# NikolayKrivosheev/Distributed-deep-learning-on-personal-computers

Hardware: AMD Instinct MI355X
Metric: images/sec (whole node), U-Net 256x256 6-class tiles (higher is better)
Workload: dtype bf16

## Files before the change

### csrc/bindings.cpp

```cpp
#include <ATen/ATen.h>
#include <c10/core/DeviceGuard.h>
#include <c10/hip/HIPStream.h>
#include <torch/library.h>

#include <cstdlib>
#include <mutex>
#include <string>
#include <unordered_map>
#include <vector>

#include "ops.h"

namespace ddlpc {

namespace {

hipStream_t cur_stream() { return c10::hip::getCurrentHIPStream().stream(); }

#define CHECK_DEV(t) TORCH_CHECK((t).is_cuda(), #t " must be a GPU tensor")
#define CHECK_CONTIG(t) TORCH_CHECK((t).is_contiguous(), #t " must be contiguous")
#define CHECK_BF16(t) TORCH_CHECK((t).scalar_type() == at::kBFloat16, #t " must be bf16")
#define CHECK_F32(t) TORCH_CHECK((t).scalar_type() == at::kFloat, #t " must be fp32")

const bf16_t* bptr(const at::Tensor& t) { return reinterpret_cast<const bf16_t*>(t.data_ptr()); }
bf16_t* bptr_mut(at::Tensor& t) { return reinterpret_cast<bf16_t*>(t.data_ptr()); }
const float* fptr_opt(const c10::optional<at::Tensor>& t) {
  return (t.has_value() && t->defined()) ? t->data_ptr<float>() : nullptr;
}

struct Geo {
  int dims, N, D, H, W, C;
};
Geo geo_of(const at::Tensor& x) {
  TORCH_CHECK(x.dim() == 4 || x.dim() == 5, "expected [N,(D,)H,W,C] channel-last tensor");
  Geo g;
  g.dims = (int)x.dim() - 2;
  g.N = (int)x.size(0);
  g.D = g.dims == 3 ? (int)x.size(1) : 1;
  g.H = (int)x.size(g.dims == 3 ? 2 : 1);
  g.W = (int)x.size(g.dims == 3 ? 3 : 2);
  g.C = (int)x.size(-1);
  return g;
}
std::vector<int64_t> shape_with_c(const Geo& g, int C, int scale = 1) {
  if (g.dims == 2) return {g.N, (int64_t)g.H * scale, (int64_t)g.W * scale, C};
  return {g.N, (int64_t)g.D * scale, (int64_t)g.H * scale, (int64_t)g.W * scale, C};
}

int pow2ceil(int v) { int p = 1; while (p < v) p <<= 1; return p; }

void conv_tile(int dims, int BM, int W, int& TD, int& TH, int& TW) {
  if (dims == 2) {
    TD = 1;
    TW = W >= 16 ? 16 : 8;
    TH = BM / TW;
  } else {
    TW = W >= 16 ? 16 : 8;
    TH = 4;
    TD = BM / (TW * TH);
  }
}

int pick_bn(int Cout) {
  if (Cout <= 32) return 32;
  if (Cout <= 64) return 64;
  return 128;
}

}

namespace {
thread_local std::string g_last_path;
}
void set_last_path(const std::string& path) { g_last_path = path; }
std::string last_path() { return g_last_path; }

namespace {
const char* const kKnobs[] = {"CROP_LDS_T", "WINDOW_LDS_T"};
bool knob_registered(const std::string& name) {
  for (const char* k : kKnobs)
    if (k[0] != 0 && name == k) return true;
  return false;
}
std::mutex g_knob_mu;
std::unordered_map<std::string, int>& knob_map() {
  static std::unordered_map<std::string, int> m;
  return m;
}
}

int knob(const char* name, int def) {
  TORCH_CHECK(knob_registered(name), "knob '", name, "' read but not listed in kKnobs");
  std::lock_guard<std::mutex> lk(g_knob_mu);
  auto& m = knob_map();
  auto it = m.find(name);
  if (it != m.end()) return it->second;
  const std::string env = std::string("DDLPC_") + name;
  const char* e = getenv(env.c_str());
  const int v = e ? atoi(e) : def;
  m.emplace(name, v);
  return v;
}

namespace {

int64_t set_knob(const std::string& name, int64_t value) {
  TORCH_CHECK(knob_registered(name), "set_knob: no kernel reads a knob named '", name,
              "' (registered knobs are listed in kKnobs, csrc/bindings.cpp)");
  std::lock_guard<std::mutex> lk(g_knob_mu);
  auto& m = knob_map();
  auto it = m.find(name);
  const int64_t prev = it != m.end() ? it->second : INT64_MIN;
  if (value == INT64_MIN) {
    if (it != m.end()) m.erase(it);
  } else {
    m[name] = (int)value;
  }
  return prev;
}

int phys_cus() {
  static int n = -1;
  if (n < 0) {
    hipDeviceProp_t prop;
    int dev = 0;
    hipGetDevice(&dev);
    n = (hipGetDeviceProperties(&prop, dev) == hipSuccess) ? prop.multiProcessorCount : 256;
  }
  return n;
}

int g_cu_reserve = 0;

int num_cus() { return std::max(8, phys_cus() - g_cu_reserve); }

at::Tensor reduce_rows(const at::Tensor& partial, int64_t R, int64_t N) {
  auto dopts = partial.options().dtype(at::kDouble);
  at::Tensor sums = at::empty({N}, dopts);
  const int RC = reduce_rows_chunks((int)R);
  at::Tensor tmp = RC > 1 ? at::empty({2 * RC * N}, dopts) : sums;
  reduce_rows_launch(partial.data_ptr<float>(), (int)R, N, tmp.data_ptr<double>(),
                     sums.data_ptr<double>(), cur_stream());
  return sums;
}

std::vector<at::Tensor> conv3_fwd(const at::Tensor& x1, const c10::optional<at::Tensor>& x2,
                                  const at::Tensor& w, const c10::optional<at::Tensor>& bias,
                                  const c10::optional<at::Tensor>& pscale,
                                  const c10::optional<at::Tensor>& pshift, int64_t cout,
                                  int64_t co1, bool want_stats_in,
                                  const c10::optional<at::Tensor>& pscale2,
                                  const c10::optional<at::Tensor>& pshift2,
                                  const c10::optional<at::Tensor>& bnb_y,
                                  const c10::optional<at::Tensor>& bnb_s4, int64_t groups) {
  CHECK_DEV(x1); CHECK_CONTIG(x1); CHECK_BF16(x1); CHECK_BF16(w); CHECK_CONTIG(w);
  c10::DeviceGuard guard(x1.device());
  const Geo g = geo_of(x1);
  bool want_stats = want_stats_in;
  ConvFwdArgs a{};
  a.dims = g.dims; a.N = g.N; a.D = g.D; a.H = g.H; a.W = g.W;
  a.C1 = g.C;
// ... 702 lines not shown
  at::Tensor out = at::empty(shape_with_c(g, (int)cout, 2), x.options());
  a.C = out.data_ptr();
  const bool res = convt_res_launch(a, num_cus(), cur_stream());
  if (!res) gemm_launch(a, cur_stream());
  set_last_path(res ? "convt_fwd:res" : "convt_fwd:gemm");
  return out;
}

std::vector<at::Tensor> convt_dgrad(const at::Tensor& dout, const at::Tensor& wd, int64_t cin,
                                    const c10::optional<at::Tensor>& bny,
                                    const c10::optional<at::Tensor>& bn4) {
  CHECK_DEV(dout); CHECK_CONTIG(dout); CHECK_BF16(dout); CHECK_BF16(wd);
  c10::DeviceGuard guard(dout.device());
  const Geo go = geo_of(dout);
  Geo g = go;
  g.H /= 2; g.W /= 2; if (g.dims == 3) g.D /= 2;
  const int S = g.dims == 2 ? 4 : 8;
  GemmArgs a{};
  a.mode = GEMM_CONVT_DGRAD;
  a.M = g.N * g.D * g.H * g.W;
  a.N = (int)cin;
  a.K = S * go.C;
  a.A = bptr(dout);
  a.B = bptr(wd);
  a.dims = g.dims; a.Nimg = g.N; a.D = g.D; a.H = g.H; a.W = g.W;
  a.Cin = (int)cin; a.Cout = go.C;
  TORCH_CHECK(go.C % 32 == 0, "convT dgrad needs Cout % 32 == 0");
  TORCH_CHECK((int64_t)a.M * (g.dims == 2 ? 4 : 8) < (int64_t)INT32_MAX, "convT: too many pixels for 32-bit pixel indices");
  at::Tensor dx = at::empty(shape_with_c(g, (int)cin), dout.options());
  a.C = dx.data_ptr();
  at::Tensor bnpart = at::empty({0}, dout.options().dtype(at::kFloat));
  a.bn4 = bn4_ptr(bn4, (int)cin);
  if (a.bn4 != nullptr) {
    TORCH_CHECK(bny.has_value() && bny->defined() && bny->is_contiguous() &&
                bny->numel() == dx.numel() && bny->scalar_type() == at::kBFloat16,
                "convt_dgrad: bny must be the deferred pre-BN input (shape of dx, bf16)");
    a.bny = bptr(*bny);
  }
  const int res_rows = convt_res_rows(a, num_cus());
  if (a.bn4 != nullptr) {
    const long long grid = res_rows > 0 ? res_rows : gemm_nt_grid(a);
    bnpart = at::empty({(int64_t)grid, 2, (int64_t)cin}, dout.options().dtype(at::kFloat));
    a.bnpart = bnpart.data_ptr<float>();
  }
  const bool res = res_rows != 0 && convt_res_launch(a, num_cus(), cur_stream());
  if (!res) gemm_launch(a, cur_stream());
  set_last_path(res ? "convt_dgrad:res" : "convt_dgrad:gemm");
  return {dx, bnpart};
}

static at::Tensor convt_bias_grad(const at::Tensor& x, const at::Tensor& dout, const Geo& go,
                                  const c10::optional<at::Tensor>& colsum_rows,
                                  const c10::optional<at::Tensor>& db_out, bool into) {
  auto fopts = x.options().dtype(at::kFloat);
  at::Tensor db = into ? *db_out : at::empty({go.C}, fopts);
  if (colsum_rows.has_value() && colsum_rows->defined() && colsum_rows->numel() > 0) {
    const at::Tensor& cr = *colsum_rows;
    TORCH_CHECK(cr.dim() == 3 && cr.size(1) == 2 && cr.size(2) >= go.C, "colsum rows [R][2][C]");
    const int R = (int)cr.size(0);
    at::Tensor ctmp = R > 64 ? at::empty({(int64_t)((R + 63) / 64) * go.C}, x.options().dtype(at::kDouble))
                             : at::empty({0}, x.options().dtype(at::kDouble));
    reduce_rows_scatter_launch(cr.data_ptr<float>(), R, go.C, ctmp.data_ptr<double>(),
                               db.data_ptr<float>(), 2, 0, 0, 0, into, cur_stream(), 2 * cr.size(2));
  } else {
    const long long P = (long long)go.N * go.D * go.H * go.W;
    const int nb = (int)std::max<long long>(1, std::min<long long>((P + 1023) / 1024, 1024));
    at::Tensor cpart = at::empty({nb, go.C}, fopts);
    channel_sum_launch(bptr(dout), P, go.C, cpart.data_ptr<float>(), nb, cur_stream());
    at::Tensor ctmp = nb > 64 ? at::empty({(int64_t)((nb + 63) / 64) * go.C},
                                          x.options().dtype(at::kDouble))
                              : at::empty({0}, x.options().dtype(at::kDouble));
    reduce_rows_scatter_launch(cpart.data_ptr<float>(), nb, go.C, ctmp.data_ptr<double>(),
                               db.data_ptr<float>(), 2, 0, 0, 0, into, cur_stream());
  }
  return db;
}

std::vector<at::Tensor> convt_wgrad(const at::Tensor& x, const at::Tensor& dout,
                                    const c10::optional<at::Tensor>& dw_out,
                                    const c10::optional<at::Tensor>& db_out,
                                    const c10::optional<at::Tensor>& colsum_rows,
                                    const c10::optional<at::Tensor>& bn4);

bool convt_bwd_fused_ok(const at::Tensor& x, const at::Tensor& dout) {
  if (x.dim() != 4 || dout.dim() != 4 || x.size(3) != 64 || dout.size(3) != 64) return false;
  if (dout.size(1) != 2 * x.size(1) || dout.size(2) != 2 * x.size(2)) return false;
  const long long K = x.size(0) * x.size(1) * x.size(2);
  if (K * 4 >= (long long)INT32_MAX) return false;
  const long long splits = std::max<long long>(1, std::min<long long>(2LL * num_cus(), K / 128));
  const long long per = (K + splits - 1) / splits + 64;
  return (4 * per + 8LL * x.size(2)) * 64 * 2 < (1LL << 31);
}

std::vector<at::Tensor> convt_bwd_fused(const at::Tensor& x, const at::Tensor& dout, const at::Tensor& wd,
                                        const c10::optional<at::Tensor>& dw_out,
                                        const c10::optional<at::Tensor>& db_out,
                                        const c10::optional<at::Tensor>& colsum_rows,
                                        const c10::optional<at::Tensor>& bn4) {
  CHECK_DEV(x); CHECK_CONTIG(x); CHECK_BF16(x); CHECK_CONTIG(dout); CHECK_BF16(dout);
  CHECK_BF16(wd); CHECK_CONTIG(wd);
  c10::DeviceGuard guard(x.device());
  const bool into = dw_out.has_value() && dw_out->defined();
  auto fopts = x.options().dtype(at::kFloat);
  if (!convt_bwd_fused_ok(x, dout)) {
    const bool has_bn = bn4.has_value() && bn4->defined();
    auto r = convt_dgrad(dout, wd, x.size(3), has_bn ? c10::optional<at::Tensor>(x) : c10::nullopt, bn4);
    auto w = convt_wgrad(x, dout, dw_out, db_out, colsum_rows, bn4);
    set_last_path("convt_bwd_fused:separate");
    return {r[0], r[1], w[0], w[1]};
  }
  TORCH_CHECK(wd.numel() == 64 * 256, "convt_bwd_fused: packed dgrad weights must be [64][256]");
  const Geo g = geo_of(x);
  const Geo go = geo_of(dout);
  GemmArgs a{};
  a.mode = GEMM_CONVT_WGRAD;
  a.M = 64; a.N = 256;
  a.K = g.N * g.H * g.W;
  a.A = bptr(x);
  a.B = bptr(dout);
  a.Wd2 = bptr(wd);
  a.dims = 2; a.Nimg = g.N; a.D = 1; a.H = g.H; a.W = g.W;
  a.Cin = 64; a.Cout = 64;
  a.bn4 = bn4_ptr(bn4, 64);
  a.splits = convt_bwd_fused_splits(a.K, num_cus());
  at::Tensor dx = at::empty_like(x);
  a.C = dx.data_ptr();
  at::Tensor part = at::empty({(int64_t)a.splits * 64 * 256}, fopts);
  a.partial = part.data_ptr<float>();
  at::Tensor bnpart = at::empty({a.bn4 != nullptr ? (int64_t)a.splits : 0, 2, 64}, fopts);
  if (a.bn4 != nullptr) a.bnpart = bnpart.data_ptr<float>();
  set_last_path("convt_bwd_fused:fused");
  convt_bwd_fused_launch(a, cur_stream());
  at::Tensor dW = into ? *dw_out : at::empty({64, 64, 2, 2}, fopts);
  const long long NW = 64LL * 256;
  at::Tensor tmp = a.splits > 64 ? at::empty({(int64_t)((a.splits + 63) / 64) * NW}, x.options().dtype(at::kDouble))
                                 : at::empty({0}, x.options().dtype(at::kDouble));
  reduce_rows_scatter_launch(part.data_ptr<float>(), a.splits, NW, tmp.data_ptr<double>(),
                             dW.data_ptr<float>(), 1, 64, 4, 64, into, cur_stream());
  at::Tensor db = convt_bias_grad(x, dout, go, colsum_rows, db_out, into);
  if (into) return {dx, bnpart, at::empty({0}, fopts), at::empty({0}, fopts)};
  return {dx, bnpart, dW, db};
}

std::vector<at::Tensor> convt_wgrad(const at::Tensor& x, const at::Tensor& dout,
                                    const c10::optional<at::Tensor>& dw_out,
                                    const c10::optional<at::Tensor>& db_out,
                                    const c10::optional<at::Tensor>& colsum_rows,
                                    const c10::optional<at::Tensor>& bn4) {
  CHECK_DEV(x); CHECK_CONTIG(x); CHECK_CONTIG(dout);
  c10::DeviceGuard guard(x.device());
  const Geo g = geo_of(x);
  const Geo go = geo_of(dout);
  const int S = g.dims == 2 ? 4 : 8;
  GemmArgs a{};
  a.mode = GEMM_CONVT_WGRAD;
  a.M = g.C;
  a.N = S * go.C;
  a.K = g.N * g.D * g.H * g.W;
  a.A = bptr(x);
  a.B = bptr(dout);
  a.dims = g.dims; a.Nimg = g.N; a.D = g.D; a.H = g.H; a.W = g.W;
  a.Cin = g.C; a.Cout = go.C;
  a.bn4 = bn4_ptr(bn4, g.C);
  int splits;
  a.wg2 = g.C % 8 == 0 && go.C % 8 == 0 && g.C <= 512;
  if (a.wg2) {
    const int tiles = convt_wgrad2_tiles(a);
    splits = std::max(1, (2 * num_cus() + tiles - 1) / tiles);
    splits = std::min(splits, std::max(1, a.K / 256));
    const long long per = ((long long)a.K + splits - 1) / splits + 64;
    const long long span = g.dims == 2 ? 4 * per + 8LL * g.W : 8 * per + 16LL * g.H * g.W;
    if (span * go.C * 2 >= (1LL << 31)) a.wg2 = 0;
  }
  if (!a.wg2) {
    const int base = ((a.M + 63) / 64) * ((a.N + 63) / 64);
    splits = std::max(1, (4 * num_cus() + base - 1) / base);
    splits = std::min(splits, std::max(1, a.K / 256));
  }
  a.splits = splits;
  auto fopts = x.options().dtype(at::kFloat);
  at::Tensor part = at::empty({(int64_t)splits * a.M * a.N}, fopts);
  a.partial = part.data_ptr<float>();
  set_last_path(a.wg2 ? "convt_wgrad:wg2" : "convt_wgrad:wg1");
  gemm_launch(a, cur_stream());
  std::vector<int64_t> ws = {g.C, go.C, 2, 2};
  if (g.dims == 3) ws.push_back(2);
  const bool into = dw_out.has_value() && dw_out->defined();
  at::Tensor dW = into ? *dw_out : at::empty(ws, fopts);
  const long long NW = (long long)a.M * a.N;
  at::Tensor tmp = splits > 64 ? at::empty({(int64_t)((splits + 63) / 64) * NW},
                                           x.options().dtype(at::kDouble))
                               : at::empty({0}, x.options().dtype(at::kDouble));
  reduce_rows_scatter_launch(part.data_ptr<float>(), splits, NW, tmp.data_ptr<double>(),
                             dW.data_ptr<float>(), 1, g.C, S, go.C, into, cur_stream());
  at::Tensor db = convt_bias_grad(x, dout, go, colsum_rows, db_out, into);
  if (into) return {at::empty({0}, fopts), at::empty({0}, fopts)};
  return {dW, db};
}

static const char* head_variant(int C) { return C == 32 ? "head32" : "split"; }

static const float* class_weight_ptr(const c10::optional<at::Tensor>& cw, const at::Tensor& a, int K) {
  if (!cw.has_value() || !cw->defined()) return nullptr;
  CHECK_F32(*cw); CHECK_CONTIG(*cw);
  TORCH_CHECK(cw->dim() == 1 && cw->numel() == K && cw->device() == a.device(),
              "class_weight must be fp32 [K] on the activation's device");
  return cw->data_ptr<float>();
}

at::Tensor head_ce_fwd(const at::Tensor& a, const at::Tensor& Wh, const at::Tensor& bh,
                       const at::Tensor& labels, int64_t ignore_index,
                       const c10::optional<at::Tensor>& bn4,
                       const c10::optional<at::Tensor>& class_weight) {
  CHECK_DEV(a); CHECK_CONTIG(a); CHECK_BF16(a); CHECK_F32(Wh); CHECK_CONTIG(Wh);
  TORCH_CHECK(labels.scalar_type() == at::kLong && labels.is_contiguous(), "labels must be int64");
  c10::DeviceGuard guard(a.device());
  const int C = (int)a.size(-1), K = (int)Wh.size(0);
  TORCH_CHECK(head_supported(C, K), "head kernel: unsupported (C, K)");
  const long long P = a.numel() / C;
  TORCH_CHECK(labels.numel() == P, "labels size mismatch");
  const int nb = (int)std::max<long long>(1, std::min<long long>((P + 255) / 256, 2048));
  auto fopts = a.options().dtype(at::kFloat);
  at::Tensor partial = at::empty({nb, 3}, fopts);
  at::Tensor out3 = at::empty({3}, fopts);
  head_ce_fwd_launch(bptr(a), Wh.data_ptr<float>(), bh.data_ptr<float>(), labels.data_ptr<int64_t>(),
                     partial.data_ptr<float>(), out3.data_ptr<float>(), bn4_ptr(bn4, C), nb, P, C, K,
                     (int)ignore_index, cur_stream(), class_weight_ptr(class_weight, a, K));
  set_last_path(std::string("head_ce_fwd:split") + (bn4_ptr(bn4, C) != nullptr ? ":defer" : ""));
  return out3;
}

std::vector<at::Tensor> head_ce_bwd(const at::Tensor& a, const at::Tensor& Wh, const at::Tensor& bh,
                                    const at::Tensor& labels, const at::Tensor& out3,
                                    const c10::optional<at::Tensor>& gscale, int64_t ignore_index,
                                    const c10::optional<at::Tensor>& dw_out,
                                    const c10::optional<at::Tensor>& db_out,
                                    const c10::optional<at::Tensor>& bn4, bool store_da,
                                    const c10::optional<at::Tensor>& class_weight) {
  CHECK_DEV(a); CHECK_CONTIG(a);
  c10::DeviceGuard guard(a.device());
  const int C = (int)a.size(-1), K = (int)Wh.size(0);
  const float* pbn = bn4_ptr(bn4, C);
  TORCH_CHECK(head_supported(C, K), "head kernel: unsupported (C, K)");
  TORCH_CHECK(store_da || pbn != nullptr, "head_ce_bwd: store_da=False needs the deferred BN (bn4)");
  const long long P = a.numel() / C;
  const int nb = head_ce_bwd_blocks(C, K, P, num_cus());
  auto fopts = a.options().dtype(at::kFloat);
  at::Tensor dA = store_da ? at::empty_like(a) : at::empty({0}, a.options());
  at::Tensor part = at::empty({nb, K * C + K}, fopts);
  at::Tensor bnpart = pbn != nullptr ? at::empty({nb, 2, C}, fopts) : at::empty({0}, fopts);
  head_ce_bwd_launch(bptr(a), Wh.data_ptr<float>(), bh.data_ptr<float>(), labels.data_ptr<int64_t>(),
                     fptr_opt(gscale), out3.data_ptr<float>(), store_da ? bptr_mut(dA) : nullptr,
                     part.data_ptr<float>(), nb, P, C, K, (int)ignore_index, pbn,
                     pbn != nullptr ? bnpart.data_ptr<float>() : nullptr, cur_stream(),
                     class_weight_ptr(class_weight, a, K));
  set_last_path(std::string("head_ce_bwd:") + head_variant(C) + (pbn != nullptr ? ":defer" : "") +
                (store_da ? "" : ":stats"));
  const bool into = dw_out.has_value() && dw_out->defined();
  at::Tensor sums = reduce_rows(part, nb, K * C + K);
  if (into) {
    TORCH_CHECK(dw_out->is_contiguous() && db_out->is_contiguous(), "grad outs must be contiguous");
    scatter_sums_launch(sums.data_ptr<double>(), K * C, dw_out->data_ptr<float>(), 2, 0, 0, 0, 1.f,
                        true, cur_stream());
    scatter_sums_launch(sums.data_ptr<double>() + K * C, K, db_out->data_ptr<float>(), 2, 0, 0, 0,
                        1.f, true, cur_stream());
    at::Tensor none = at::empty({0}, fopts);
// ... 809 lines not shown
```

### csrc/convt_gemm.hip

```cpp
#include <type_traits>

#include "common.h"
#include "conv_lds.h"
#include "ops.h"

namespace ddlpc {

namespace {

constexpr int BK = 32;
DDLPC_DEVICE int swz(int row, int chunk) { return chunk ^ (((row >> 2) & 1) << 1); }
DDLPC_DEVICE int lds_off(int row, int chunk) { return row * 64 + (swz(row, chunk) << 4); }

DDLPC_DEVICE int up_pixel(int m, int sub, int dims, int D, int H, int W) {
  const int q = udiv_pow2(m, W), w = m - q * W;
  if (dims == 2) {
    const int i = sub >> 1, j = sub & 1;
    return (2 * q + i) * (2 * W) + 2 * w + j;
  }
  const int q2 = udiv_pow2(q, H), h = q - q2 * H;
  const int kd = sub >> 2, i = (sub >> 1) & 1, j = sub & 1;
  (void)D;
  return ((2 * q2 + kd) * (2 * H) + 2 * h + i) * (2 * W) + 2 * w + j;
}
// ... 798 lines not shown
          uint4* q = reinterpret_cast<uint4*>(sA(buf) + ((i * 4 + wave) * 64 + lane) * 16);
          float f[8];
          unpack8(*q, f);
#pragma unroll
          for (int j = 0; j < 8; ++j) f[j] = fmaxf(fmaf(f[j], s_bn[a_col[i] + j], s_bn[NBF + a_col[i] + j]), 0.f);
          *q = pack8(f);
        }
      }
    };
    const int g = lane >> 4, q = (lane & 15) >> 2, pp = lane & 3;
    auto frag_off = [&](int row, int col, auto rb_tag) {
      constexpr int RB = decltype(rb_tag)::value;
      const int grp = (col >> 4) ^ tn2_swz<RB>(row);
      return row * RB + grp * 32 + (col & 15) * 2;
    };
    using RA = std::integral_constant<int, Cf::A_RB>;
    using RBt = std::integral_constant<int, Cf::B_RB>;
    const int nst = (int)((k_end - k_begin + KT - 1) / KT);
    __syncthreads();
#pragma unroll
    for (int j = 0; j < NBUF - 1; ++j)
      if (j < nst) issue(k_begin + (long long)j * KT, j);
    constexpr int PER = Cf::NA + Cf::NB;
#pragma unroll 1
    for (int st = 0; st < nst; ++st) {
      const int buf = st % NBUF;
      const long long k0 = k_begin + (long long)st * KT;
      if constexpr (NBUF == 2) {
        if (st + 1 < nst) { issue(k0 + KT, buf ^ 1); dma_wait<PER>(); }
        else dma_wait<0>();
        if (has_bn) transform(k0, buf);
        lds_sync();
      } else {
        const int after = min(NBUF - 2, nst - 1 - st);
        if (NBUF >= 4 && after >= 2) dma_wait<2 * PER>();
        else if (after >= 1) dma_wait<PER>();
        else dma_wait<0>();
        if (has_bn) transform(k0, buf);
        lds_sync();
        if (st + NBUF - 1 < nst) issue(k0 + (long long)(NBUF - 1) * KT, (st + NBUF - 1) % NBUF);
      }
      const char* A_ = sA(buf);
      const char* B_ = sB(buf);
#pragma unroll
      for (int ks = 0; ks < KT / 32; ++ks) {
      const int r0 = ks * 32 + 8 * g + q;
      uint4 af[4], bfr[4];
#pragma unroll
      for (int mt = 0; mt < 4; ++mt) {
        const int c = wm * 64 + mt * 16 + 4 * pp;
        const uint2 lo = lds_read_tr16(A_ + frag_off(r0, c, RA{}));
        const uint2 hi = lds_read_tr16(A_ + frag_off(r0 + 4, c, RA{}));
        af[mt] = make_uint4(lo.x, lo.y, hi.x, hi.y);
      }
#pragma unroll
      for (int nt = 0; nt < 4; ++nt) {
        const int c = wn * 64 + nt * 16 + 4 * pp;
        const uint2 lo = lds_read_tr16(B_ + frag_off(r0, c, RBt{}));
        const uint2 hi = lds_read_tr16(B_ + frag_off(r0 + 4, c, RBt{}));
        bfr[nt] = make_uint4(lo.x, lo.y, hi.x, hi.y);
      }
#pragma unroll
      for (int mt = 0; mt < 4; ++mt)
#pragma unroll
        for (int nt = 0; nt < 4; ++nt) acc[mt][nt] = mfma16x16x32(af[mt], bfr[nt], acc[mt][nt]);
      }
      if (NBUF == 2) lds_sync();
    }
  }
  float* out = p.partial + (long long)split * p.M * p.N;
#pragma unroll
  for (int mt = 0; mt < 4; ++mt)
#pragma unroll
    for (int nt = 0; nt < 4; ++nt) {
      const int n = n0 + wn * 64 + nt * 16 + (lane & 15);
#pragma unroll
      for (int i = 0; i < 4; ++i) {
        const int m = m0 + wm * 64 + mt * 16 + 4 * (lane >> 4) + i;
        if (m < p.M && n < p.N) out[(long long)m * p.N + n] = acc[mt][nt][i];
      }
    }
}

struct FbCfg {
  static constexpr int KT = 32, A_RB = 128, B_RB = 512;
  static constexpr int A_BYTES = KT * A_RB, B_BYTES = KT * B_RB;
  static constexpr int NA = A_BYTES / 4096, NB = B_BYTES / 4096;
  static constexpr int STAGE = A_BYTES + B_BYTES;
  static constexpr int WD_BYTES = 64 * 512;
  static constexpr int SMEM = 2 * STAGE + WD_BYTES + 4 * 64 * 4;
};

__global__ __launch_bounds__(256, 2) void convt_bwd_fused_kernel(GemmArgs p) {
  using namespace convlds;
  using Cf = FbCfg;
  constexpr int KT = Cf::KT, PER = Cf::NA + Cf::NB;
  extern __shared__ __attribute__((aligned(16))) char smem[];
  char* sWd = smem + 2 * Cf::STAGE;
  float* s_bn = reinterpret_cast<float*>(sWd + Cf::WD_BYTES);
  auto sA = [&](int b) { return smem + b * Cf::STAGE; };
  auto sB = [&](int b) { return smem + b * Cf::STAGE + Cf::A_BYTES; };
  const int tid = threadIdx.x, lane = tid & 63;
  const int wave = __builtin_amdgcn_readfirstlane(tid >> 6);
  const bool has_bn = p.bn4 != nullptr;
  if (has_bn && tid < 64) {
    const float is = p.bn4[64 + tid];
    s_bn[tid] = p.bn4[128 + tid];
    s_bn[64 + tid] = p.bn4[192 + tid];
    s_bn[128 + tid] = is;
    s_bn[192 + tid] = -p.bn4[tid] * is;
  }
  const int split = xcd_remap(blockIdx.x, gridDim.x);
  const long long npx = (long long)p.K;
  const long long per = ((npx + p.splits - 1) / p.splits + KT - 1) / KT * KT;
  const long long k_begin = per * split;
  const long long k_end = k_begin + per < npx ? k_begin + per : npx;
  f32x4_t acc[4][4];
#pragma unroll
  for (int i = 0; i < 4; ++i)
#pragma unroll
    for (int j = 0; j < 4; ++j) acc[i][j] = f32x4_t{0.f, 0.f, 0.f, 0.f};
  float bs1[4] = {0.f, 0.f, 0.f, 0.f}, bs2[4] = {0.f, 0.f, 0.f, 0.f};
  const int g = lane >> 4, q = (lane & 15) >> 2, pp = lane & 3;
  const int ci4 = 16 * wave + 4 * g;
  if (k_begin < k_end) {
    const long long a_lo = k_begin;
    const auto ra = make_rsrc(p.A + a_lo * 64, (unsigned)((k_end - a_lo) * 64 * 2));
    const long long kb0 = k_begin - k_begin % p.W;
    const long long b_lo = up_pixel((int)kb0, 0, 2, 1, p.H, p.W);
    const long long b_hi = (long long)up_pixel((int)(k_end - 1), 3, 2, 1, p.H, p.W) + 1;
    const auto rb = make_rsrc(p.B + b_lo * 64, (unsigned)((b_hi - b_lo) * 64 * 2));
    const auto rx = make_rsrc(static_cast<bf16_t*>(p.C) + a_lo * 64, (unsigned)((k_end - a_lo) * 64 * 2));
    {
      const auto rw = make_rsrc(p.Wd2, 64 * 256 * 2);
#pragma unroll
      for (int i = 0; i < 8; ++i) {
        const int e = (i * 4 + wave) * 64 + lane;
        const int row = e >> 5, pc = e & 31;
        dma16(rw, sWd + (i * 4 + wave) * 1024, (unsigned)((row * 256 + ((pc ^ (row & 15)) * 8)) * 2));
      }
    }
    int a_row, a_col, b_row[Cf::NB], b_col[Cf::NB], b_sub[Cf::NB];
    {
      const int e = wave * 64 + lane;
      const int row = e / 8, pc = e % 8;
      a_row = row;
      a_col = ((((pc >> 1) ^ tn2_swz<Cf::A_RB>(row)) << 1) | (pc & 1)) * 8;
    }
#pragma unroll
    for (int i = 0; i < Cf::NB; ++i) {
      const int e = (i * 4 + wave) * 64 + lane;
      const int row = e / 32, pc = e % 32;
      const int n = ((((pc >> 1) ^ tn2_swz<Cf::B_RB>(row)) << 1) | (pc & 1)) * 8;
      b_row[i] = row;
      b_sub[i] = n >> 6;
      b_col[i] = n & 63;
    }
    auto issue = [&](long long k0, int buf) {
      {
        const long long px = k0 + a_row;
        dma16(ra, sA(buf) + wave * 1024, px < k_end ? (unsigned)(((px - a_lo) * 64 + a_col) * 2) : kOOB);
      }
#pragma unroll
      for (int i = 0; i < Cf::NB; ++i) {
        const long long px = k0 + b_row[i];
        const bool ok = px < k_end;
// ... 61 lines not shown
#pragma unroll
        for (int nt = 0; nt < 4; ++nt) {
          const int c = wave * 64 + nt * 16 + 4 * pp;
          const uint2 lo = lds_read_tr16(B_ + frag_off(r0, c, RBt{}));
          const uint2 hi = lds_read_tr16(B_ + frag_off(r0 + 4, c, RBt{}));
          bfr[nt] = make_uint4(lo.x, lo.y, hi.x, hi.y);
        }
#pragma unroll
        for (int mt = 0; mt < 4; ++mt)
#pragma unroll
          for (int nt = 0; nt < 4; ++nt) acc[mt][nt] = mfma16x16x32(af[mt], bfr[nt], acc[mt][nt]);
      }
      f32x4_t dacc[2] = {f32x4_t{0.f, 0.f, 0.f, 0.f}, f32x4_t{0.f, 0.f, 0.f, 0.f}};
      {
        const int wrow = 16 * wave + (lane & 15);
#pragma unroll
        for (int kk = 0; kk < 8; ++kk) {
          const int lp = 4 * kk + g;
          const uint4 aw = lds128(sWd + wrow * 512 + ((lp ^ (wrow & 15)) << 4));
#pragma unroll
          for (int t = 0; t < 2; ++t) {
            const int prow = 16 * t + (lane & 15);
            const uint4 bx = lds128(B_ + prow * 512 + ((((lp >> 1) ^ tn2_swz<Cf::B_RB>(prow)) << 1 | (lp & 1)) << 4));
            dacc[t] = mfma16x16x32(aw, bx, dacc[t]);
          }
        }
      }
#pragma unroll
      for (int t = 0; t < 2; ++t) {
        const int prow = 16 * t + (lane & 15);
        const long long px = k0 + prow;
        const bool ok = px < k_end;
        const uint32_t lo = pack2(dacc[t][0], dacc[t][1]), hi = pack2(dacc[t][2], dacc[t][3]);
        __builtin_amdgcn_raw_buffer_store_b64(u32x2_t{lo, hi}, rx,
                                              ok ? (unsigned)(((px - a_lo) * 64 + ci4) * 2) : kOOB, 0, 0);
        if (has_bn && ok) {
          const uint2 yv = *reinterpret_cast<const uint2*>(A_ + frag_off(prow, ci4, RA{}));
          const float d[4] = {lo_bf(lo), hi_bf(lo), lo_bf(hi), hi_bf(hi)};
          const float y[4] = {lo_bf(yv.x), hi_bf(yv.x), lo_bf(yv.y), hi_bf(yv.y)};
#pragma unroll
          for (int i = 0; i < 4; ++i) {
            const float a = fmaf(y[i], ysc[i], ysh[i]);
            const float dyh = a > 0.f ? d[i] : 0.f;
            const float xh = fmaf(y[i], yis[i], ynm[i]);
            bs1[i] += dyh;
            bs2[i] = fmaf(dyh, xh, bs2[i]);
          }
        }
      }
      lds_sync();
    }
  }
  float* out = p.partial + (long long)split * 64 * 256;
#pragma unroll
  for (int mt = 0; mt < 4; ++mt)
#pragma unroll
    for (int nt = 0; nt < 4; ++nt) {
      const int n = wave * 64 + nt * 16 + (lane & 15);
#pragma unroll
      for (int i = 0; i < 4; ++i) out[(long long)(mt * 16 + 4 * g + i) * 256 + n] = acc[mt][nt][i];
    }
  if (has_bn) {
#pragma unroll
    for (int o = 1; o < 16; o <<= 1)
#pragma unroll
      for (int i = 0; i < 4; ++i) { bs1[i] += __shfl_xor(bs1[i], o, 64); bs2[i] += __shfl_xor(bs2[i], o, 64); }
    if ((lane & 15) == 0) {
      float* row = p.bnpart + (long long)split * 128;
#pragma unroll
      for (int i = 0; i < 4; ++i) { row[ci4 + i] = bs1[i]; row[64 + ci4 + i] = bs2[i]; }
    }
  }
}

}

void convt_bwd_fused_launch(GemmArgs& a, hipStream_t st) {
  hipLaunchKernelGGL(convt_bwd_fused_kernel, dim3(a.splits), dim3(256), FbCfg::SMEM, st, a);
}
int convt_bwd_fused_splits(long long K, int num_cus) {
  return (int)std::max<long long>(1, std::min<long long>(2LL * num_cus, K / 128));
}

int convt_wgrad2_tiles(const GemmArgs& a) {
  const int bm = a.M <= 64 ? 64 : 128;
  const int bn = bm == 64 ? 256 : 128;
  return ((a.M + bm - 1) / bm) * ((a.N + bn - 1) / bn);
}

int gemm_nt_bn(const GemmArgs& a) {
  return a.N % 128 == 0 ? 128 : 64;
}

long long gemm_nt_grid(const GemmArgs& a) {
  if (gemm_nt_dgrad2_ok(a)) return ((a.M + Dg2Cfg::BM - 1) / Dg2Cfg::BM) * (long long)(a.N / Dg2Cfg::BN);
  const int bn = gemm_nt_bn(a);
  return ((a.M + 127) / 128) * (long long)((a.N + bn - 1) / bn);
}

void gemm_launch(GemmArgs& a, hipStream_t st) {
  if (a.mode == GEMM_CONVT_WGRAD && a.wg2) {
    const int grid = convt_wgrad2_tiles(a) * a.splits;
    if (a.M <= 64)
      hipLaunchKernelGGL(gemm_tn_wgrad2_kernel<64>, dim3(grid), dim3(256), Tn2Cfg<64>::SMEM, st, a);
    else
      hipLaunchKernelGGL(gemm_tn_wgrad2_kernel<128>, dim3(grid), dim3(256), Tn2Cfg<128>::SMEM, st, a);
    return;
  }
  if (a.mode == GEMM_CONVT_WGRAD) {
    const int grid = ((a.M + 63) / 64) * ((a.N + 63) / 64) * a.splits;
    hipLaunchKernelGGL(gemm_tn_wgrad_kernel, dim3(grid), dim3(256), 0, st, a);
    return;
  }
  if (gemm_nt_fwd2_mode(a)) {
    const bool w256 = a.N % 256 == 0 && a.M >= 65536;
    const int bnt = w256 ? 256 : 128;
    const int ntn = a.N / bnt;
    const long long mt = (a.M + 255) / 256;
    const long long rneed = (mt + 7) / 8;
    const int per_cu = w256 ? 1 : 2;
    const int R = (int)std::max<long long>(1, std::min<long long>(rneed, (long long)per_cu * device_cus() / (8 * ntn)));
    const unsigned grid2 = (unsigned)(8 * R * ntn);
    if (w256)
      hipLaunchKernelGGL((gemm_nt_fwd2_kernel<1, 256>), dim3(grid2), dim3(512), (Nt2Cfg<1, 256>::SMEM), st, a);
    else
      hipLaunchKernelGGL((gemm_nt_fwd2_kernel<1>), dim3(grid2), dim3(512), Nt2Cfg<1>::SMEM, st, a);
    return;
  }
  if (gemm_nt_dgrad2_ok(a)) {
    hipLaunchKernelGGL(gemm_nt_dgrad2_kernel, dim3((unsigned)gemm_nt_grid(a)), dim3(512), Dg2Cfg::SMEM, st, a);
    return;
  }
  const int bn = gemm_nt_bn(a);
  const long long grid = gemm_nt_grid(a);
  const int kc = a.mode == GEMM_CONVT_FWD ? 1 : a.K <= 64 ? 2 : 4;
  if (a.mode == GEMM_CONVT_FWD) {
    if (bn == 128) hipLaunchKernelGGL((gemm_nt_kernel<GEMM_CONVT_FWD, 1, 128>), dim3((unsigned)grid), dim3(256), 0, st, a);
    else hipLaunchKernelGGL((gemm_nt_kernel<GEMM_CONVT_FWD, 1, 64>), dim3((unsigned)grid), dim3(256), 0, st, a);
  } else if (bn == 128) {
    if (kc == 2) hipLaunchKernelGGL((gemm_nt_kernel<GEMM_CONVT_DGRAD, 2, 128>), dim3((unsigned)grid), dim3(256), 0, st, a);
    else hipLaunchKernelGGL((gemm_nt_kernel<GEMM_CONVT_DGRAD, 4, 128>), dim3((unsigned)grid), dim3(256), 0, st, a);
  } else if (kc == 2) {
    hipLaunchKernelGGL((gemm_nt_kernel<GEMM_CONVT_DGRAD, 2, 64>), dim3((unsigned)grid), dim3(256), 0, st, a);
  } else {
    hipLaunchKernelGGL((gemm_nt_kernel<GEMM_CONVT_DGRAD, 4, 64>), dim3((unsigned)grid), dim3(256), 0, st, a);
  }
}

}
```

### csrc/ops.h

```cpp
#pragma once

#include <hip/hip_runtime.h>
#include <stdint.h>

#include <algorithm>
#include <string>

#include "common.h"

namespace ddlpc {

struct ConvFwdArgs {
  int dims;
  int N, D, H, W;
  int C1, C2, Cin, CinW;
  int Cout, Co1;
  int taps;
  const bf16_t* X1;
  const bf16_t* X2;
  const float* pscale;
  const float* pshift;
  const float* pscale2;
  const float* pshift2;
  const bf16_t* Wt;
// ... 27 lines not shown
int conv3_fwd_cfg_halo(int dims, int cfg);

struct Bwd32Args {
  int N, H, W;
  const bf16_t* dY;
  const bf16_t* Y;
  const float* s4;
  const bf16_t* Wd;
  bf16_t* dA;
  float* bnpart;
  float* wpart;
  int tilesH, tilesW, nTiles;
  int groups;
};
int conv3_bwd32_grid(int nTiles, int num_cus, int groups);
void conv3_bwd32_launch(const Bwd32Args& a, int grid, hipStream_t st);

struct ConvWgradArgs {
  int dims;
  int N, D, H, W;
  int C1, C2, Cin, Cout, taps;
  const bf16_t* dY;
  const bf16_t* X1;
  const bf16_t* X2;
  const float* pscale;
  const float* pshift;
  const float* pscale2;
  const float* pshift2;
  float* partial;
  int TD, TH, TW;
  int tilesD, tilesH, tilesW, nTiles;
  int coTiles, ciChunks, planes, splits;
  const bf16_t* dyy;
  const float* dys4;
  const float* dycoef;
  bf16_t* dyout;
  int ciw;
  int groups;
  int gimg;
  long long gstride;
};
void conv3_wgrad_launch(ConvWgradArgs& a, int bco, hipStream_t st);
int conv3d_wgrad_ds_plan(ConvWgradArgs& a, int num_cus);
void conv3d_wgrad_ds_launch(ConvWgradArgs& a, int grid, hipStream_t st);
int conv3_wgrad_c32_plan(ConvWgradArgs& a, int num_cus);
void conv3_wgrad_c32_launch(ConvWgradArgs& a, int grid, hipStream_t st);
void conv3_wgrad2_launch(ConvWgradArgs& a, int bco, hipStream_t st);
int conv3_wgrad2_pt(int bco, int C2, int H, int W);
void conv3_wgrad3_launch(ConvWgradArgs& a, int bco, hipStream_t st);
void conv3_wgrad_img_launch(ConvWgradArgs& a, int bco, hipStream_t st);
int conv3_wgrad_img_pt(int bco);

int conv3_wgrad_halo_cap(int dims);

struct GemmArgs {
  int mode;
  int M, N, K;
  const bf16_t* A;
  const bf16_t* B;
  const float* bias;
  void* C;
  float* partial;
  int splits;
  int dims, Nimg, D, H, W;
  int Cin, Cout;
  const float* pscale;
  const float* pshift;
  const float* bn4;
  const bf16_t* bny;
  float* bnpart;
  int wg2;
  const bf16_t* Wd2;
};
enum GemmMode {
  GEMM_CONVT_FWD = 0,
  GEMM_CONVT_DGRAD = 1,
  GEMM_CONVT_WGRAD = 2,
};
void gemm_launch(GemmArgs& a, hipStream_t st);
int convt_bwd_fused_splits(long long K, int num_cus);
int gemm_nt_bn(const GemmArgs& a);
long long gemm_nt_grid(const GemmArgs& a);
int convt_wgrad2_tiles(const GemmArgs& a);
void convt_bwd_fused_launch(GemmArgs& a, hipStream_t st);
int convt_res_rows(const GemmArgs& a, int num_cus);
bool convt_res_launch(GemmArgs& a, int num_cus, hipStream_t st);


const char* bn_relu_apply_launch(const bf16_t* y, const float* scale, const float* shift, bf16_t* out,
                                 bf16_t* pooled, int dims, int N, int D, int H, int W, int C,
                                 hipStream_t st, int groups = 1, long long sstride = 0);
void bn_bwd_reduce_launch(const bf16_t* dA, const bf16_t* dP, const bf16_t* y,
                          const float* scale, const float* shift, const float* mean,
                          const float* invstd, const float* gscale, float* partial, int nblocks,
                          int dims, int N, int D, int H, int W, int C, hipStream_t st);
const char* bn_bwd_apply_launch(const bf16_t* dA, const bf16_t* dP, const bf16_t* y, const float* scale,
                                const float* shift, const float* mean, const float* invstd,
                                const float* coefs, const float* gscale, bf16_t* dY, int dims, int N,
                                int D, int H, int W, int C, hipStream_t st);
int bn_bwd_reduce_blocks(long long pixels_or_quads);
bool bn_group_supported(int dims, bool pool, int D, int H, int W, int C);
int bn_group_stats_rows(long long gpix, int C, int groups);
void bn_group_stats_finalize_launch(const bf16_t* y, int groups, long long gpix, int C,
                                    const float* gamma, const float* beta, float eps, float* out4,
                                    float* arena, long long astride, float* partial_scratch,
                                    int nb, hipStream_t st);
int bn_group_bwd_rows(long long items_per_group, int groups);
const char* bn_group_backward_launch(const bf16_t* dA, const bf16_t* dP, const bf16_t* y,
                                     const float* stats4, const float* gamma, float* dgamma, float* dbeta,
                                     bool accumulate, float* coefs, float* partial_scratch, int nb,
                                     bf16_t* dY, int dims, int groups, int N, int D, int H, int W, int C,
                                     hipStream_t st, bool have_partial, double* gsum_scratch);
void bn_group_grad_rows_launch(const float* partial, int nb, int groups, int C, double count,
                               const float* gamma, const float* stats4, float* dgamma, float* dbeta,
                               bool accumulate, float* coefs, double* gsum_scratch,
                               const float* dscale, hipStream_t st);
void bn_group_finalize_rows_launch(const float* partial, int nb, int groups, long long gpix, int C,
                                   const float* gamma, const float* beta, float eps, float* out4,
                                   float* arena, long long astride, hipStream_t st);

bool head_supported(int C, int K);
void head_ce_fwd_launch(const bf16_t* a, const float* Wh, const float* bh, const int64_t* labels,
                        float* partial, float* out3, const float* bn4, int nblocks, long long P,
                        int C, int K, int ignore_index, hipStream_t st, const float* cw = nullptr);
int head_ce_bwd_blocks(int C, int K, long long P, int num_cus);
int head_fwd_stats_blocks(int C, int K, long long P, int num_cus, int groups = 1);
void head_ce_bwd_launch(const bf16_t* a, const float* Wh, const float* bh, const int64_t* labels,
                        const float* gscale, const float* stats3, bf16_t* dA, float* dW_partial,
                        int nblocks, long long P, int C, int K, int ignore_index, const float* bn4,
                        float* bnpart, hipStream_t st, const float* cw = nullptr);
void head_ce_fwd_stats_launch(const bf16_t* a, const float* Wh, const float* bh,
                              const int64_t* labels, const float* bn4, float* dW_partial,
                              float* bnpart, float* loss_partial, float* out3, int nblocks,
                              long long P, int C, int K, int ignore_index, hipStream_t st,
                              int groups = 1, const float* cw = nullptr);
void head_bn_apply_launch(const bf16_t* a, const float* Wh, const float* bh, const int64_t* labels,
                          const float* gscale, const float* stats3, const float* bn4,
                          const float* coefs, bf16_t* dY, long long P, int C, int K,
                          int ignore_index, int num_cus, hipStream_t st, int groups = 1,
                          const float* cw = nullptr);
void head_logits_launch(const bf16_t* a, const float* Wh, const float* bh, float* logits_nchw,
                        long long P, long long HW, int C, int K, const float* bn4, hipStream_t st);
void head_predict_accum_launch(const bf16_t* a, const float* Wh, const float* bh, const int* origins,
                               const float* win, float* acc, int B, int S, uint32_t codes, int tile,
                               int H, int W, int KA, int C, int K, const float* bn4, hipStream_t st);

int window_gather_blocks(int tile);
void window_gather_launch(const uint8_t* scene, const int* origins, int B, int S, uint32_t codes,
                          int H, int W, int in_ch, int tile, int cpad, bool lds_transpose, bf16_t* x,
                          hipStream_t st);
void scene_finalize_launch(const float* acc, long long P, int K, int KA, const uint8_t* labels,
                           int ignore_index, uint8_t* pred, int64_t* cm, hipStream_t st);

void adam_launch(float* p, const float* g, float* m, float* v, long long n, float b1, float b2,
                 float eps, float wd, float step_size, float inv_sqrt_bc2, hipStream_t st,
                 const float* dscal = nullptr);
void adam_scalars_launch(float* s, double lr, double b1, double b2, hipStream_t st);
struct PackEntry {
  const float* src;
  bf16_t* fwd;
  bf16_t* dgrad;
  int kind;
  int Cout, Cin, taps, CinW, CoutW;
};
void weight_pack_launch(const PackEntry* entries_dev, int n_entries, long long max_elems,
                        hipStream_t st);
// ... 81 lines not shown
```

Baseline: 7938.

## Add wide-tile 512-thread transposed-conv weight-gradient kernel for large channel counts

Adds a new weight-gradient GEMM kernel for 2D transposed convolutions that uses 256-wide N tiles, 128 or 256-row M tiles, 8 waves and a 4-deep LDS pipeline. A shape-based rule (or a knob override) selects it for large M/N layers and uses fewer K-splits, which reduces partial-sum traffic and raises data reuse per tile. It costs more LDS and registers per block, and may lower occupancy or parallelism on smaller K.

After: 8031, median of 6. 1.2% higher.

```diff
diff --git a/csrc/bindings.cpp b/csrc/bindings.cpp
--- a/csrc/bindings.cpp
+++ b/csrc/bindings.cpp
@@ -76,7 +76,7 @@
 std::string last_path() { return g_last_path; }
 
 namespace {
-const char* const kKnobs[] = {"CROP_LDS_T", "WINDOW_LDS_T"};
+const char* const kKnobs[] = {"CROP_LDS_T", "WINDOW_LDS_T", "CONVT_WGRAD_WIDE"};
 bool knob_registered(const std::string& name) {
   for (const char* k : kKnobs)
     if (k[0] != 0 && name == k) return true;
@@ -945,6 +945,13 @@
                                     const c10::optional<at::Tensor>& colsum_rows,
                                     const c10::optional<at::Tensor>& bn4);
 
+static bool convt_wgrad_wide_rule(const GemmArgs& a) {
+  const bool bn = a.bn4 != nullptr;
+  if (a.M == 256 && a.N == 1024) return a.K >= (bn ? 16384 : 65536);
+  if (a.M == 128 && a.N == 512) return bn && a.K >= 131072;
+  return false;
+}
+
 bool convt_bwd_fused_ok(const at::Tensor& x, const at::Tensor& dout) {
   if (x.dim() != 4 || dout.dim() != 4 || x.size(3) != 64 || dout.size(3) != 64) return false;
   if (dout.size(1) != 2 * x.size(1) || dout.size(2) != 2 * x.size(2)) return false;
@@ -1028,12 +1035,21 @@
   int splits;
   a.wg2 = g.C % 8 == 0 && go.C % 8 == 0 && g.C <= 512;
   if (a.wg2) {
-    const int tiles = convt_wgrad2_tiles(a);
-    splits = std::max(1, (2 * num_cus() + tiles - 1) / tiles);
-    splits = std::min(splits, std::max(1, a.K / 256));
-    const long long per = ((long long)a.K + splits - 1) / splits + 64;
-    const long long span = g.dims == 2 ? 4 * per + 8LL * g.W : 8 * per + 16LL * g.H * g.W;
-    if (span * go.C * 2 >= (1LL << 31)) a.wg2 = 0;
+    const int kw = knob("CONVT_WGRAD_WIDE", -1);
+    auto plan = [&]() {
+      const int tiles = convt_wgrad2_tiles(a);
+      splits = a.wg2 == 2 ? std::max(1, num_cus() / tiles)
+                          : std::max(1, (2 * num_cus() + tiles - 1) / tiles);
+      splits = std::min(splits, std::max(1, a.K / 256));
+      const long long per = ((long long)a.K + splits - 1) / splits + 64;
+      const long long span = g.dims == 2 ? 4 * per + 8LL * g.W : 8 * per + 16LL * g.H * g.W;
+      return span * go.C * 2 < (1LL << 31) && (a.wg2 != 2 || per * g.C * 2 < (1LL << 31));
+    };
+    if (kw != 0 && convt_wgrad2w_ok(a) && (kw == 1 || convt_wgrad_wide_rule(a))) {
+      a.wg2 = 2;
+      if (!plan()) a.wg2 = 1;
+    }
+    if (a.wg2 == 1 && !plan()) a.wg2 = 0;
   }
   if (!a.wg2) {
     const int base = ((a.M + 63) / 64) * ((a.N + 63) / 64);
@@ -1044,7 +1060,7 @@
   auto fopts = x.options().dtype(at::kFloat);
   at::Tensor part = at::empty({(int64_t)splits * a.M * a.N}, fopts);
   a.partial = part.data_ptr<float>();
-  set_last_path(a.wg2 ? "convt_wgrad:wg2" : "convt_wgrad:wg1");
+  set_last_path(a.wg2 == 2 ? "convt_wgrad:wg2w" : a.wg2 ? "convt_wgrad:wg2" : "convt_wgrad:wg1");
   gemm_launch(a, cur_stream());
   std::vector<int64_t> ws = {g.C, go.C, 2, 2};
   if (g.dims == 3) ws.push_back(2);
diff --git a/csrc/convt_gemm.hip b/csrc/convt_gemm.hip
--- a/csrc/convt_gemm.hip
+++ b/csrc/convt_gemm.hip
@@ -904,6 +904,203 @@
     }
 }
 
+template <int BM>
+struct Tn2wCfg {
+  static constexpr int BN = 256, KT = 32, NBUF = 4, NWAVE = 8;
+  static constexpr int WM = BM / 2;
+  static constexpr int MT = WM / 16;
+  static constexpr int A_RB = BM * 2, B_RB = BN * 2;
+  static constexpr int A_BYTES = KT * A_RB, B_BYTES = KT * B_RB;
+  static constexpr int NA = A_BYTES / (NWAVE * 1024);
+  static constexpr int NB = B_BYTES / (NWAVE * 1024);
+  static constexpr int STAGE = A_BYTES + B_BYTES;
+  static constexpr int BN_FLOATS = 512;
+  static constexpr int SMEM = NBUF * STAGE + 2 * BN_FLOATS * 4;
+};
+
+template <int BM>
+__global__ __launch_bounds__(512) void gemm_tn_wgrad2w_kernel(GemmArgs p) {
+  using namespace convlds;
+  using Cf = Tn2wCfg<BM>;
+  constexpr int BN = Cf::BN, KT = Cf::KT, NBUF = Cf::NBUF, NBF = Cf::BN_FLOATS, MT = Cf::MT;
+  extern __shared__ __attribute__((aligned(16))) char smem[];
+  float* s_bn = reinterpret_cast<float*>(smem + NBUF * Cf::STAGE);
+  auto sA = [&](int b) { return smem + b * Cf::STAGE; };
+  auto sB = [&](int b) { return smem + b * Cf::STAGE + Cf::A_BYTES; };
+  const int tid = threadIdx.x, lane = tid & 63;
+  const int wave = __builtin_amdgcn_readfirstlane(tid >> 6);
+  const int wm = wave >> 2, wn = wave & 3;
+  const bool has_bn = p.bn4 != nullptr;
+  if (has_bn)
+    for (int i = tid; i < p.M; i += 512) { s_bn[i] = p.bn4[2 * p.M + i]; s_bn[NBF + i] = p.bn4[3 * p.M + i]; }
+  const int nTilesN = (p.N + BN - 1) / BN, nTilesM = (p.M + BM - 1) / BM;
+  int b = xcd_remap(blockIdx.x, gridDim.x);
+  const int ntile = b % nTilesN; b /= nTilesN;
+  const int mtile = b % nTilesM; b /= nTilesM;
+  const int split = b;
+  const int m0 = mtile * BM, n0 = ntile * BN;
+  const long long npx = (long long)p.K;
+  const long long per = ((npx + p.splits - 1) / p.splits + 63) / 64 * 64;
+  const long long k_begin = per * split;
+  const long long k_end = k_begin + per < npx ? k_begin + per : npx;
+  f32x4_t acc[MT][4];
+#pragma unroll
+  for (int i = 0; i < MT; ++i)
+#pragma unroll
+    for (int j = 0; j < 4; ++j) acc[i][j] = f32x4_t{0.f, 0.f, 0.f, 0.f};
+  if (k_begin < k_end) {
+    const long long a_lo = k_begin;
+    const auto ra = make_rsrc(p.A + a_lo * p.Cin, (unsigned)((k_end - a_lo) * p.Cin * 2));
+    const long long kb0 = k_begin - k_begin % p.W;
+    const long long b_lo = up_pixel((int)kb0, 0, 2, 1, p.H, p.W);
+    const long long b_hi = (long long)up_pixel((int)(k_end - 1), 3, 2, 1, p.H, p.W) + 1;
+    const auto rb = make_rsrc(p.B + b_lo * p.Cout, (unsigned)((b_hi - b_lo) * p.Cout * 2));
+    int a_row[Cf::NA], a_col[Cf::NA], b_row[Cf::NB], b_col[Cf::NB], b_sub[Cf::NB];
+#pragma unroll
+    for (int i = 0; i < Cf::NA; ++i) {
+      const int e = (i * 8 + wave) * 64 + lane;
+      constexpr int ppr = Cf::A_RB / 16;
+      const int row = e / ppr, pc = e % ppr;
+      const int lp = (((pc >> 1) ^ tn2_swz<Cf::A_RB>(row)) << 1) | (pc & 1);
+      a_row[i] = row;
+      a_col[i] = m0 + lp * 8 < p.M ? m0 + lp * 8 : -1;
+    }
+#pragma unroll
+    for (int i = 0; i < Cf::NB; ++i) {
+      const int e = (i * 8 + wave) * 64 + lane;
+      constexpr int ppr = Cf::B_RB / 16;
+      const int row = e / ppr, pc = e % ppr;
+      const int lp = (((pc >> 1) ^ tn2_swz<Cf::B_RB>(row)) << 1) | (pc & 1);
+      const int n = n0 + lp * 8;
+      b_row[i] = row;
+      b_sub[i] = n < p.N ? n / p.Cout : -1;
+      b_col[i] = n < p.N ? n % p.Cout : 0;
+    }
+    int b_w[Cf::NB], b_base[Cf::NB], b_so[Cf::NB];
+    const int W = p.W, dq = KT / W, dw = KT % W, dbase = 4 * W * dq + 2 * dw;
+#pragma unroll
+    for (int i = 0; i < Cf::NB; ++i) {
+      const long long px0 = k_begin + b_row[i];
+      const int qq = (int)(px0 / W);
+      b_w[i] = (int)(px0 - (long long)qq * W);
+      b_base[i] = 4 * qq * W + 2 * b_w[i];
+      b_so[i] = b_sub[i] >= 0 ? (b_sub[i] >> 1) * 2 * W + (b_sub[i] & 1) : 0;
+    }
+    auto issue = [&](long long k0, int buf) {
+#pragma unroll
+      for (int i = 0; i < Cf::NA; ++i) {
+        const long long px = k0 + a_row[i];
+        const bool ok = px < k_end && a_col[i] >= 0;
+        dma16(ra, sA(buf) + (i * 8 + wave) * 1024,
+              ok ? (unsigned)(((px - a_lo) * p.Cin + a_col[i]) * 2) : kOOB);
+      }
+#pragma unroll
+      for (int i = 0; i < Cf::NB; ++i) {
+        const long long px = k0 + b_row[i];
+        const bool ok = px < k_end && b_sub[i] >= 0;
+        const long long up = ok ? (long long)(b_base[i] + b_so[i]) : b_lo;
+        b_w[i] += dw;
+        b_base[i] += dbase;
+        if (b_w[i] >= W) { b_w[i] -= W; b_base[i] += 2 * W; }
+        dma16(rb, sB(buf) + (i * 8 + wave) * 1024,
+              ok ? (unsigned)(((up - b_lo) * p.Cout + b_col[i]) * 2) : kOOB);
+      }
+    };
+    __syncthreads();
+    float bsc[Cf::NA][8], bsh[Cf::NA][8];
+#pragma unroll
+    for (int i = 0; i < Cf::NA; ++i) {
+      const int c = has_bn && a_col[i] >= 0 ? a_col[i] : 0;
+#pragma unroll
+      for (int h = 0; h < 2; ++h) {
+        const float4 s = *reinterpret_cast<const float4*>(s_bn + c + 4 * h);
+        const float4 t = *reinterpret_cast<const float4*>(s_bn + NBF + c + 4 * h);
+        bsc[i][4 * h] = s.x; bsc[i][4 * h + 1] = s.y; bsc[i][4 * h + 2] = s.z; bsc[i][4 * h + 3] = s.w;
+        bsh[i][4 * h] = t.x; bsh[i][4 * h + 1] = t.y; bsh[i][4 * h + 2] = t.z; bsh[i][4 * h + 3] = t.w;
+      }
+    }
+    auto transform = [&](long long k0, char* __restrict__ A) __attribute__((always_inline)) {
+#pragma unroll
+      for (int i = 0; i < Cf::NA; ++i) {
+        if (k0 + a_row[i] < k_end && a_col[i] >= 0) {
+          uint4* q = reinterpret_cast<uint4*>(A + ((i * 8 + wave) * 64 + lane) * 16);
+          float f[8];
+          unpack8(*q, f);
+#pragma unroll
+          for (int j = 0; j < 8; ++j) f[j] = fmaxf(fmaf(f[j], bsc[i][j], bsh[i][j]), 0.f);
+          *q = pack8(f);
+        }
+      }
+    };
+    const int g = lane >> 4, q = (lane & 15) >> 2, pp = lane & 3;
+    auto frag_off = [&](int row, int col, auto rb_tag) {
+      constexpr int RB = decltype(rb_tag)::value;
+      const int grp = (col >> 4) ^ tn2_swz<RB>(row);
+      return row * RB + grp * 32 + (col & 15) * 2;
+    };
+    using RA = std::integral_constant<int, Cf::A_RB>;
+    using RBt = std::integral_constant<int, Cf::B_RB>;
+    const int r0 = 8 * g + q;
+    const int nst = (int)((k_end - k_begin + KT - 1) / KT);
+    constexpr int PER = Cf::NA + Cf::NB;
+#pragma unroll
+    for (int j = 0; j < NBUF - 1; ++j)
+      if (j < nst) issue(k_begin + (long long)j * KT, j);
+    auto compute = [&](const char* __restrict__ A_, const char* __restrict__ B_) __attribute__((always_inline)) {
+      uint4 af[MT], bfr[4];
+#pragma unroll
+      for (int mt = 0; mt < MT; ++mt) {
+        const int c = wm * Cf::WM + mt * 16 + 4 * pp;
+        const uint2 lo = lds_read_tr16(A_ + frag_off(r0, c, RA{}));
+        const uint2 hi = lds_read_tr16(A_ + frag_off(r0 + 4, c, RA{}));
+        af[mt] = make_uint4(lo.x, lo.y, hi.x, hi.y);
+      }
+#pragma unroll
+      for (int nt = 0; nt < 4; ++nt) {
+        const int c = wn * 64 + nt * 16 + 4 * pp;
+        const uint2 lo = lds_read_tr16(B_ + frag_off(r0, c, RBt{}));
+        const uint2 hi = lds_read_tr16(B_ + frag_off(r0 + 4, c, RBt{}));
+        bfr[nt] = make_uint4(lo.x, lo.y, hi.x, hi.y);
+      }
+#pragma unroll
+      for (int mt = 0; mt < MT; ++mt)
+#pragma unroll
+        for (int nt = 0; nt < 4; ++nt) acc[mt][nt] = mfma16x16x32(af[mt], bfr[nt], acc[mt][nt]);
+    };
+    auto stage = [&](int st) __attribute__((always_inline)) {
+      const int buf = st % NBUF;
+      const long long k0 = k_begin + (long long)st * KT;
+      if (has_bn) transform(k0, sA(buf));
+      lds_sync();
+      if (st + NBUF - 1 < nst) issue(k0 + (long long)(NBUF - 1) * KT, (st + NBUF - 1) % NBUF);
+      compute(sA(buf), sB(buf));
+    };
+    int st = 0;
+#pragma unroll 1
+    for (; st < nst - (NBUF - 2); ++st) {
+      dma_wait<(NBUF - 2) * PER>();
+      stage(st);
+    }
+#pragma unroll 1
+    for (; st < nst; ++st) {
+      vm_wait_dyn((nst - 1 - st) * PER);
+      stage(st);
+    }
+  }
+  float* out = p.partial + (long long)split * p.M * p.N;
+#pragma unroll
+  for (int mt = 0; mt < MT; ++mt)
+#pragma unroll
+    for (int nt = 0; nt < 4; ++nt) {
+      const int n = n0 + wn * 64 + nt * 16 + (lane & 15);
+#pragma unroll
+      for (int i = 0; i < 4; ++i) {
+        const int m = m0 + wm * Cf::WM + mt * 16 + 4 * (lane >> 4) + i;
+        if (m < p.M && n < p.N) out[(long long)m * p.N + n] = acc[mt][nt][i];
+      }
+    }
+}
+
 struct FbCfg {
   static constexpr int KT = 32, A_RB = 128, B_RB = 512;
   static constexpr int A_BYTES = KT * A_RB, B_BYTES = KT * B_RB;
@@ -1131,7 +1328,15 @@
   return (int)std::max<long long>(1, std::min<long long>(2LL * num_cus, K / 128));
 }
 
+bool convt_wgrad2w_ok(const GemmArgs& a) {
+  return a.mode == GEMM_CONVT_WGRAD && a.dims == 2 && a.M >= 128 && a.M <= 512 && a.N >= 256;
+}
+
 int convt_wgrad2_tiles(const GemmArgs& a) {
+  if (a.wg2 == 2) {
+    const int bm = a.M >= 256 ? 256 : 128;
+    return ((a.M + bm - 1) / bm) * ((a.N + 255) / 256);
+  }
   const int bm = a.M <= 64 ? 64 : 128;
   const int bn = bm == 64 ? 256 : 128;
   return ((a.M + bm - 1) / bm) * ((a.N + bn - 1) / bn);
@@ -1150,7 +1355,11 @@
 void gemm_launch(GemmArgs& a, hipStream_t st) {
   if (a.mode == GEMM_CONVT_WGRAD && a.wg2) {
     const int grid = convt_wgrad2_tiles(a) * a.splits;
-    if (a.M <= 64)
+    if (a.wg2 == 2 && a.M >= 256)
+      hipLaunchKernelGGL(gemm_tn_wgrad2w_kernel<256>, dim3(grid), dim3(512), Tn2wCfg<256>::SMEM, st, a);
+    else if (a.wg2 == 2)
+      hipLaunchKernelGGL(gemm_tn_wgrad2w_kernel<128>, dim3(grid), dim3(512), Tn2wCfg<128>::SMEM, st, a);
+    else if (a.M <= 64)
       hipLaunchKernelGGL(gemm_tn_wgrad2_kernel<64>, dim3(grid), dim3(256), Tn2Cfg<64>::SMEM, st, a);
     else
       hipLaunchKernelGGL(gemm_tn_wgrad2_kernel<128>, dim3(grid), dim3(256), Tn2Cfg<128>::SMEM, st, a);
diff --git a/csrc/ops.h b/csrc/ops.h
--- a/csrc/ops.h
+++ b/csrc/ops.h
@@ -133,6 +133,7 @@
 int gemm_nt_bn(const GemmArgs& a);
 long long gemm_nt_grid(const GemmArgs& a);
 int convt_wgrad2_tiles(const GemmArgs& a);
+bool convt_wgrad2w_ok(const GemmArgs& a);
 void convt_bwd_fused_launch(GemmArgs& a, hipStream_t st);
 int convt_res_rows(const GemmArgs& a, int num_cus);
 bool convt_res_launch(GemmArgs& a, int num_cus, hipStream_t st);
```
